# NoelShin/zutis

Hardware: AMD Instinct MI355X
Metric: images/sec, COCO2017-val-shaped ViT-B/16 dense semantic segmentation @336px (ZUTIS forward + semantic predict), batches of 32 per GPU, 3 independent batches in flight (higher is better)
Workload: dtype f16x3 (fp32-class)

## Files before the change

include/zutis_hip.h:

```cpp
#ifndef ZUTIS_HIP_H
#define ZUTIS_HIP_H

#include <stddef.h>

#ifdef __cplusplus
extern "C" {
#endif

typedef struct ihipStream_t* zh_stream_t;

#define ZH_OK 0
#define ZH_ERR_ARG (-1)
#define ZH_ERR_HIP (-2)
#define ZH_ERR_WORKSPACE (-3)

#define ZH_ACT_NONE 0
#define ZH_ACT_QUICKGELU 1
#define ZH_ACT_RELU 2
#define ZH_ACT_SIGMOID 3
#define ZH_ACT_GELU_ERF 4

#define ZH_ABI_VERSION 233
int zh_version(void);
const char* zh_arch(void);
const char* zh_last_error(void);

int zh_dev_set_gemm_overrides(int group_m, int tile, int tile_small);

int zh_dev_set_gemm_persist(int workgroups);

int zh_gemm_f16(const void* A, long lda, long strideA, const void* W, long ldw, long strideW,
                void* C, long ldc, long strideC, int out_f16,
                const float* bias, const float* residual, long ldr, long strideR, int res_rows,
                const void* pos_y, const void* pos_x, long ld_pos, int pos_h, int pos_w, int pos_f16,
                int act, int M, int N, int K, int batch, zh_stream_t stream);

int zh_gemm_f16_res16(const void* A, long lda, long strideA, const void* W, long ldw, long strideW,
                      void* C, long ldc, long strideC,
                      const float* bias, const void* residual, long ldr, long strideR, int res_rows,
                      int M, int N, int K, int batch, zh_stream_t stream);

#define ZH_GEMM_FIXED_K_ORDER 1
int zh_gemm_f16x3(const void* A, long lda, long strideA, long planeA, const void* W, long ldw, long strideW, long planeW,
                  void* C, long ldc, long strideC, long planeC, int out_kind, float out_scale,
                  const float* bias, const float* residual, long ldr, long strideR, int res_rows,
                  const void* pos_y, const void* pos_x, long ld_pos, int pos_h, int pos_w, int pos_f16,
                  int act, int M, int N, int K, int batch, int flags, zh_stream_t stream);

size_t zh_attention_splitk_workspace_size(int batch, int heads, int Tq, int head_dim, int ksplit);
int zh_attention_f16_splitk(const void* Q, long ldq, long strideQ, const void* K, long ldk, long strideK,
                            const void* V, long ldv, long strideV, void* O, long ldo, long strideO,
                            int batch, int heads, int Tq, int Tk, int head_dim, float scale,
                            long planeQ, long planeK, long planeV, long planeO, int ksplit, void* workspace, size_t workspace_bytes,
                            zh_stream_t stream);
int zh_attention_f16(const void* Q, long ldq, long strideQ, const void* K, long ldk, long strideK,
                     const void* V, long ldv, long strideV, void* O, long ldo, long strideO,
                     int batch, int heads, int Tq, int Tk, int head_dim, float scale,
                     long planeQ, long planeK, long planeV, long planeO, zh_stream_t stream);

int zh_attention_causal_f16(const void* Q, long ldq, long strideQ, const void* K, long ldk, long strideK,
                            const void* V, long ldv, long strideV, void* O, long ldo, long strideO,
                            int batch, int heads, int T, int head_dim, float scale,
                            long planeQ, long planeK, long planeV, long planeO, zh_stream_t stream);

int zh_embed_tokens_f32(const long long* tokens, const float* table, const float* pos, float* out, long n, int ctx, int D,
                        int vocab, zh_stream_t stream);
int zh_eot_rows_f32(const long long* tokens, const float* x, float* out, long n, int ctx, int D, zh_stream_t stream);
int zh_group_mean_l2norm(const float* x, float* out, int groups, int T, int E, zh_stream_t stream);

int zh_layernorm_f32(const float* x, long in_group_rows, long in_group_stride, long in_offset,
                     long out_group_rows, long out_group_stride, long out_offset,
                     const float* gamma, const float* beta, float eps,
                     float* out_f32, void* out_f16, void* out_f16_plus, float* out_f32_plus,
                     const float* add, int add_rows, int rows, int D, long lo_plane, int* status, zh_stream_t stream);
int zh_layernorm_f16(const void* x, long in_group_rows, long in_group_stride, long in_offset,
                     long out_group_rows, long out_group_stride, long out_offset,
                     const float* gamma, const float* beta, float eps,
                     float* out_f32, void* out_f16, void* out_f16_plus, float* out_f32_plus,
                     const float* add, int add_rows, int rows, int D, long lo_plane, int* status, zh_stream_t stream);
#define ZH_STATUS_RANGE 1
#define ZH_STATUS_NONFINITE 2
#define ZH_STATUS_LABEL 4

int zh_sum_layernorm_f32(const float* parts, int n_parts, long part_stride, const float* bias, const float* residual,
                         float* out_sum, const float* gamma, const float* beta, float eps,
                         float* out_f32, void* out_f16, long lo_plane,
                         long out_group_rows, long out_group_stride, long out_offset, int skip_first_in_group,
                         const float* gamma2, const float* beta2, float eps2, float* out2_f32, void* out2_f16, long lo_plane2,
                         long out2_group_rows, long out2_group_stride, long out2_offset,
                         int rows, int D, int* status, zh_stream_t stream);

int zh_assemble_tokens_ln(const float* patch_emb, const float* class_embedding, const float* pos_embed,
                          const float* gamma, const float* beta, float eps, float* out,
                          int B, int T, int D, zh_stream_t stream);

int zh_assemble_tokens_ln_f16(const float* patch_emb, const float* class_embedding, const float* pos_embed,
                              const float* gamma, const float* beta, float eps, void* out,
                              int B, int T, int D, zh_stream_t stream);

int zh_l2norm_rows(const float* x, float* out_f32, void* out_f16, float eps, int rows, int D, long lo_plane, float f16_scale, zh_stream_t stream);

size_t zh_global_ln_l2_workspace_size(int B, int M, int C);
int zh_global_ln_l2(const float* x, float* out_f32, void* out_f16, float eps, float l2_eps,
                    int B, int M, int C, void* workspace, size_t workspace_bytes, long lo_plane, float f16_scale, int* status,
                    zh_stream_t stream);

int zh_im2col_f16(const float* x, void* out, int B, int Cin, int H, int W, int patch, int Kpad, int pad_to_patch,
                  long lo_plane, zh_stream_t stream);

int zh_posembed_bicubic(const float* pos, float* out, int grid, int h, int w, int D, float scale_h, float scale_w,
                        int has_cls, zh_stream_t stream);

int zh_upsample2x_bilinear_cl(const float* x, float* out_f32, void* out_f16, int B, int h, int w, int D, long lo_plane,
                              int relu, zh_stream_t stream);

int zh_sine_pe(float* out, int h, int w, int D, float temperature, zh_stream_t stream);

int zh_add_rowperiodic_f16(const void* a, const float* add, void* out, long rows, int D, int add_rows, long a_lo_plane,
                           long lo_plane, zh_stream_t stream);

int zh_fill_f32(float* x, float value, long n, zh_stream_t stream);

int zh_cast_f32_f16(const float* x, const float* add, int add_rows, void* out, long rows, int D, long lo_plane, float f16_scale,
                    zh_stream_t stream);

int zh_upsample_argmax(const float* logits_lo, long long* labels, int B, int n, int h, int w, int H, int W,
                       float scale_h, float scale_w, zh_stream_t stream);

#define ZH_GT_U8 0
#define ZH_GT_RG16 1
int zh_upsample_argmax_score(const float* logits_lo, const unsigned char* gt, int gt_format, long long* hist_accum,
                             long long* labels, int B, int n, int h, int w, int H, int W, float scale_h, float scale_w,
                             zh_stream_t stream);

int zh_upsample_argmax_bytes(const float* logits_lo, unsigned char* labels_out, int label_format, unsigned char* overlay_out,
                             const unsigned char* packed, const int* desc, const unsigned char* palette, int alpha,
                             int B, int n, int h, int w, int H, int W, float scale_h, float scale_w, zh_stream_t stream);

int zh_upsample_bilinear_nchw(const float* x, float* out, unsigned char* mask_u8, float threshold, long planes,
                              int h, int w, int H, int W, float scale_h, float scale_w, zh_stream_t stream);

int zh_select_upsample_mask(const float* objectness, const float* masks, unsigned char* out_u8, long long* index, int B, int Q,
                            int h, int w, int H, int W, float scale_h, float scale_w, float threshold, zh_stream_t stream);

int zh_resize_nearest_u8(const unsigned char* x, unsigned char* out, int h, int w, int H, int W, float scale_h, float scale_w,
                         zh_stream_t stream);

int zh_confusion_hist(const long long* label_true, const long long* label_pred, long long* hist_accum, long total,
                      int n_class, zh_stream_t stream);

int zh_instance_mask_stats(const float* mask_proposals, long stride_image, float threshold, int B, int Q, int M,
                           float* sizes, float* confidence, unsigned char* binary, int* range_flag, zh_stream_t stream);
size_t zh_masked_mean_workspace_size(int B, int Q, int M, int E);
int zh_masked_mean_tokens(const float* tokens, const unsigned char* binary, const float* sizes, float* avg,
                          int B, int Q, int M, int E, void* workspace, size_t workspace_bytes, zh_stream_t stream);
int zh_instance_classify(const float* avg, const float* text, const float* confidence, float temperature,
                         int rows, int n_classes, int E, long long* category, float* score, zh_stream_t stream);
size_t zh_mask_iou_workspace_size(int n, long pixels);
int zh_mask_iou_counts(const unsigned char* masks, int n, long pixels, int* inter, int* uni,
                       void* workspace, size_t workspace_bytes, zh_stream_t stream);

#define ZH_RCN_KMAX 152
int zh_resize_crop_normalize_u8(const unsigned char* packed, long packed_bytes, const int* desc, int B, int n_px, int kmax,
                                const float* lut, float* out, zh_stream_t stream);
#define ZH_FILTER_BILINEAR 2
#define ZH_FILTER_BICUBIC 3
int zh_resize_normalize_u8(const unsigned char* packed, long packed_bytes, const int* desc, int B, int out_h, int out_w, int filter,
                           int kmax, const float* lut, float* out, zh_stream_t stream);

int zh_denormalize_u8(const float* x, unsigned char* rgb, int H, int W, const float* mean3, const float* std3,
                      zh_stream_t stream);
int zh_bgrid_coords(const unsigned char* rgb, int H, int W, double sigma_spatial, double sigma_luma, double sigma_chroma,
                    int* coords, zh_stream_t stream);
size_t zh_bilateral_workspace_size(int H, int W, double sigma_spatial, double sigma_luma, double sigma_chroma);
int zh_bilateral_solve(const unsigned char* rgb, const unsigned char* target_u8, const double* target_f64, int H, int W,
                       double sigma_spatial, double sigma_luma, double sigma_chroma, double confidence, double lam,
                       double a_diag_min, double cg_tol, int cg_maxiter, double* out_soft, int* stats,
                       double* n_out, double* m_out, void* workspace, size_t workspace_bytes, zh_stream_t stream);

int zh_bilateral_solve_batch(const unsigned char* rgb, const unsigned char* target_u8, const double* target_f64, int B, int H, int W,
                             double sigma_spatial, double sigma_luma, double sigma_chroma, double confidence, double lam,
                             double a_diag_min, double cg_tol, int cg_maxiter, double* out_soft, int* stats,
                             double* n_out, double* m_out, void* workspace, size_t workspace_bytes, zh_stream_t stream);

int zh_threshold_f64_u8(const double* x, double threshold, unsigned char* out, long n, zh_stream_t stream);

int zh_topk_rows(const float* scores, long ld, int rows, long N, int k, const long long* idx_map, long long idx_add,
                 long long* idx_out, float* val_out, long out_ld, zh_stream_t stream);

int zh_mask_nms(const int* inter, const int* uni, const float* scores, const long long* category_ids, int B, int Q,
                int nms_type, double nms_threshold, double sigma, double score_threshold,
                int* out_index, double* out_score, long long* out_category, int* out_count, double* packed, const int* range_flag,
                int* zero_word, zh_stream_t stream);

size_t zh_mask_runs_workspace_size(int n, int W);
int zh_mask_runs(const unsigned char* masks, const int* sel, int n_sel, int H, int W, int max_runs,
                 int* positions, int* nruns, int* box_area, void* workspace, size_t workspace_bytes, zh_stream_t stream);
int zh_mask_runs_kept(const unsigned char* masks, const int* kept_index, const int* kept_count, int B, int Q, int H, int W, int max_runs,
                      int* positions, long packed_capacity, int* nruns, int* box_area, void* workspace, size_t workspace_bytes,
                      zh_stream_t stream);

int zh_mask_rle_kept(const int* positions, long packed_capacity, const int* nruns, const int* kept_count, int B, int Q, int max_runs, long HW,
                     unsigned char* out, long out_capacity, int* out_len, zh_stream_t stream);

int zh_mask_rle_fused_supported(int H, int W, int max_runs);
int zh_mask_rle_fused_kept(const unsigned char* masks, const unsigned long long* bits, const int* kept_index, const int* kept_count, int B, int Q,
                           int H, int W, int max_runs, unsigned char* out, long out_capacity, int* cursor, int* info, zh_stream_t stream);

size_t zh_mask_match_cost_workspace_size(int B, int L, int Q, int H, int n_max);
int zh_mask_match_cost(const float* proposals, const unsigned char* gt_u8, const int* inst_off, float* costs, float* stat_p,
                       float* stat_pg, float* stat_g, int* skip, int* status, int B, int L, int Q, int h, int w, int H, int W,
                       int n_max, float weight_dice, float weight_bce, float scale_h, float scale_w, void* workspace,
                       size_t workspace_bytes, zh_stream_t stream);
int zh_mask_match_grad(const float* proposals, const unsigned char* gt_u8, const int* inst_off, const int* pairs, int n_pairs,
                       const float* stat_p, const float* stat_pg, const float* stat_g, const float* grad_out, float* grad_proposals,
                       int B, int L, int Q, int h, int w, int H, int W, float weight_dice, float weight_bce, float loss_scale,
                       float scale_h, float scale_w, zh_stream_t stream);
size_t zh_upsample_ce_workspace_size(int B, int H, int W);
int zh_upsample_ce_fwd(const float* logits_lo, const long long* labels, float* lse, float* out, int* status, int B, int n_cat,
                       int h, int w, int H, int W, int ignore_index, float scale_h, float scale_w, void* workspace,
                       size_t workspace_bytes, zh_stream_t stream);
int zh_upsample_ce_bwd(const float* logits_lo, const long long* labels, const float* lse, const float* ce_out,
                       const float* grad_out, float* grad_logits_lo, int B, int n_cat, int h, int w, int H, int W,
                       int ignore_index, float scale_h, float scale_w, zh_stream_t stream);
int zh_gemm_f32_strided(const float* A, long sAb, long sAm, long sAk, const float* Bm, long sBb, long sBn, long sBk, float* C,
                        long sCb, long sCm, long sCn, int batch, int M, int N, int K, zh_stream_t stream);

int zh_linear_assignment_max_dim(void);
size_t zh_linear_assignment_workspace_size(int B, int L, int n_tot);
int zh_linear_assignment(const float* costs, const int* inst_off, const int* skip, int B, int L, int Q, int n_max, int n_tot,
                         int* pairs, int* n_pairs, float* mask_loss, int* status, void* workspace, size_t workspace_bytes,
                         zh_stream_t stream);
int zh_pack_masks_u8(const void* const* src, const int* counts, int B, int elem_size, long HW, unsigned char* gt_u8, int* inst_off,
                     zh_stream_t stream);

int zh_plan_run(const void* cmds, int n, zh_stream_t stream);
int zh_plan_run2(const void* cmds_a, int na, zh_stream_t stream_a, const void* cmds_b, int nb, zh_stream_t stream_b);
int zh_plan_run_multi(const void* const* cmds, const int* n, const zh_stream_t* streams, int count);
const char* zh_plan_op_name(int op);

long zh_rle_counts_to_string_host(const long long* counts, long n, char* out, long cap);
long zh_rle_from_transitions_host(const int* positions, long stride, int packed, const int* nruns, long n, long HW, char* out, long cap,
                                  long long* offsets);

int zh_synth_geometry_u8(const unsigned char* packed, long packed_bytes, const int* desc, int N, int C, int ignore_index, int kmax,
                         int fill_w, int fill_h, int* work, unsigned char* out_rgbm, zh_stream_t stream);
int zh_synth_photometric_u8(unsigned char* rgbm, const int* desc, int N, int C, int* work, zh_stream_t stream);
int zh_synth_blur_u8(const unsigned char* rgbm, const int* desc, const float* weights, int N, int C, int ksize, unsigned char* out_rgbm,
                     zh_stream_t stream);
int zh_synth_compose(const unsigned char* rgbm, const unsigned char* rgbm_blurred, const int* desc, const int* samples, const int* work,
                     const float* lut, int N, int B, int C, int ignore_index, float* image, long long* semantic, unsigned char* onehot,
                     zh_stream_t stream);

long zh_rle_encode_host(const unsigned char* mask, int H, int W, char* out, long cap);

#ifdef __cplusplus
}
#endif
#endif
```

zutis_amd/build.py:

```python
from __future__ import annotations

import os
import subprocess
import sys

HERE = os.path.dirname(os.path.abspath(__file__))
CSRC = os.path.join(HERE, "csrc")
LIB = os.path.join(HERE, "libzutis_hip.so")
EXTRA_FLAGS = {"bilateral.hip": ["-ffp-contract=off"], "preprocess.hip": ["-ffp-contract=off"],
               "synth.hip": ["-ffp-contract=off"]}
NO_SCRATCH = {"gemm.hip", "gemm_x3.hip", "attention.hip", "preprocess.hip", "synth.hip", "resample.hip"}
MAX_SCRATCH = int(os.environ.get("ZH_BUILD_MAX_SCRATCH", "0"))
MIN_OCCUPANCY = {"attention.hip": {"attn_f16_kernelILi64ELi4ELi1ELi0EE": 3, "attn_f16_kernelILi64ELi4ELi0ELi0EE": 3,
                                   "attn_f16_kernelILi64ELi4ELi1ELi1EE": 2, "attn_f16_kernelILi96ELi4ELi1ELi0EE": 2,
                                   "attn_f16_kernelILi96ELi4ELi0ELi0EE": 2, "attn_f16_kernelILi96ELi4ELi1ELi1EE": 2},
                 "resample.hip": {"upsample_argmax_pk_kernelI7UaBytes": 3, "upsample_argmax_lds_kernelI7UaBytes": 6,
                                  "upsample_argmax_kernelI7UaBytes": 8}}
SOURCES = ["capi.hip", "gemm.hip", "gemm_x3.hip", "attention.hip", "norm.hip", "resample.hip", "metrics.hip", "instance.hip", "bilateral.hip", "preprocess.hip", "retrieval.hip", "text.hip", "criterion.hip", "assign.hip", "synth.hip", "plan.hip"]


def _hipcc() -> str:
    for c in (os.environ.get("HIPCC"), "/opt/rocm/bin/hipcc", "hipcc"):
        if c and (os.path.isabs(c) and os.path.exists(c) or not os.path.isabs(c)):
            return c
    raise RuntimeError("hipcc not found")


def sources():
    return [os.path.join(CSRC, s) for s in SOURCES if os.path.exists(os.path.join(CSRC, s))]


def needs_build() -> bool:
    if not os.path.exists(LIB):
        return True
    t = os.path.getmtime(LIB)
    deps = sources() + [os.path.join(CSRC, "common.h"), os.path.join(CSRC, "gemm_kernel.h"), os.path.join(CSRC, "gemm_skinny.h"),
                        os.path.join(CSRC, "rcn.h"), os.path.join(os.path.dirname(HERE), "include", "zutis_hip.h")]
    return any(os.path.getmtime(d) > t for d in deps)


def build(force: bool = False, verbose: bool = True) -> str:
    if not force and not needs_build():
        return LIB
    objs = []
    os.makedirs(os.path.join(HERE, "_obj"), exist_ok=True)
    from . import plan
    plan.generate_dispatch(os.path.join(CSRC, "plan_gen.inc"))
    procs = []
    for src in sources():
        obj = os.path.join(HERE, "_obj", os.path.basename(src)[:-4] + ".o")
        objs.append(obj)
        deps = [src, os.path.join(CSRC, "common.h")]
        if os.path.basename(src).startswith("gemm"):
            deps.append(os.path.join(CSRC, "gemm_kernel.h"))
            deps.append(os.path.join(CSRC, "gemm_skinny.h"))
        if os.path.basename(src) in ("preprocess.hip", "synth.hip"):
            deps.append(os.path.join(CSRC, "rcn.h"))
        if os.path.basename(src) in ("plan.hip", "capi.hip"):
            deps.append(os.path.join(os.path.dirname(HERE), "include", "zutis_hip.h"))
        if not force and os.path.exists(obj) and all(os.path.getmtime(obj) > os.path.getmtime(d) for d in deps):
            continue
        cmd = [_hipcc(), "--offload-arch=gfx950", "-O3", "-fPIC", "-std=c++17"] + EXTRA_FLAGS.get(os.path.basename(src), []) + \
              ["-c", src, "-o", obj]
        if os.path.basename(src) in NO_SCRATCH:
            cmd.insert(1, "-Rpass-analysis=kernel-resource-usage")
        if verbose:
            print(" ".join(cmd), flush=True)
        procs.append((cmd, src, subprocess.Popen(cmd, stderr=subprocess.PIPE, text=True)))
    for cmd, src, p in procs:
        _, err = p.communicate()
        if p.returncode != 0:
            sys.stderr.write(err)
            raise RuntimeError("hipcc failed: " + " ".join(cmd))
        if os.path.basename(src) in NO_SCRATCH:
            spills = [ln for ln in err.splitlines() if "ScratchSize [bytes/lane]:" in ln
                      and int(ln.split("ScratchSize [bytes/lane]:")[1].split()[0]) > MAX_SCRATCH]
            if spills:
                raise RuntimeError(f"{os.path.basename(src)}: a kernel spills to scratch (register budget exceeded): {spills[0].strip()}")
            fn = None
            min_occ = MIN_OCCUPANCY.get(os.path.basename(src), {})
            matched = set()
            for ln in err.splitlines():
                if "Function Name:" in ln:
                    fn = ln.split("Function Name:")[1].split()[0]
                elif "Occupancy [waves/SIMD]:" in ln and fn:
                    occ = int(ln.split("Occupancy [waves/SIMD]:")[1].split()[0])
                    for key, need in min_occ.items():
                        if key in fn:
                            matched.add(key)
                            if occ < need:
                                raise RuntimeError(f"{os.path.basename(src)}: {fn} compiles to {occ} waves/SIMD, its design needs {need}")
            unmatched = sorted(set(min_occ) - matched)
            if unmatched:
                raise RuntimeError(f"{os.path.basename(src)}: MIN_OCCUPANCY names no kernel of the compiler's remarks: {', '.join(unmatched)}")
        else:
            sys.stderr.write(err)
    cmd = [_hipcc(), "--offload-arch=gfx950", "-shared", "-fPIC", "-o", LIB] + objs
    if verbose:
        print(" ".join(cmd), flush=True)
    subprocess.check_call(cmd)
    return LIB


if __name__ == "__main__":
    print(build(force="--force" in sys.argv))
```

zutis_amd/csrc/attention.hip:

```cpp
#include "common.h"
#include <type_traits>

struct AttnArgs {
  const half_t* Q; long ldq, sQ;
  const half_t* K; long ldk, sK;
  const half_t* V; long ldv, sV;
  half_t* O; long ldo, sO;
  int Tq, Tk, H, nqb, groups;
  float scale_log2;
  int causal;
  long planeQ, planeK, planeV, planeO;
  int ksplit, kchunk;
  float* part_o; float* part_m; float* part_l;
};

typedef __fp16 fp16x4 __attribute__((__vector_size__(4 * sizeof(__fp16))));
typedef __attribute__((address_space(3))) fp16x4* lds_fp16x4_ptr;

#define KT 64
#define VS 96

#define ZH_ATTN_LAZY_LOG2 8.0f

__device__ __forceinline__ float zh_xor32_max(float x) {
  float a = x, b = x;
  asm volatile("s_nop 1\n\tv_permlane32_swap_b32 %0, %1" : "+v"(a), "+v"(b));
  float r;
  asm("v_max_f32 %0, %1, %2" : "=v"(r) : "v"(a), "v"(b));
  return r;
}
__device__ __forceinline__ float zh_xor32_sum(float x) {
  float a = x, b = x;
  asm volatile("s_nop 1\n\tv_permlane32_swap_b32 %0, %1" : "+v"(a), "+v"(b));
  return a + b;
}

template <int DH, int NWAVE, int X3, int PIPE>
__global__ __launch_bounds__(64 * NWAVE, X3 ? 2 : (DH == 64 ? 3 : 2)) void attn_f16_kernel(AttnArgs p) {
  static_assert(!PIPE || X3, "the pipelined loop exists for the split-pair kernels");
  constexpr int NT = 64 * NWAVE;
  constexpr int KS = DH + 8;
  constexpr int NKS = DH / 16;
  constexpr int NDT = DH / 32;
  constexpr int CPR = DH / 8;
  constexpr int KTT = X3 ? 32 : KT;
  constexpr int NU = KTT / 32;
  constexpr int NLD = (KTT * CPR + NT - 1) / NT;
  constexpr bool LDFULL = (KTT * CPR) % NT == 0;
  __shared__ __attribute__((aligned(16))) half_t sKb[2][KTT * KS];
  __shared__ __attribute__((aligned(16))) half_t sKl[X3 ? 2 : 1][X3 ? KTT * KS : 8];
  __shared__ __attribute__((aligned(16))) half_t sVb[2][KTT * VS];
  __shared__ __attribute__((aligned(16))) half_t sVl[X3 ? 2 : 1][X3 ? KTT * VS : 8];

  const int tid = threadIdx.x, lane = tid & 63, wave = tid >> 6;
  const int id = blockIdx.y * gridDim.x + blockIdx.x;
  const int per_group = p.nqb * p.ksplit;
  const int item = (id & 7) * (int)(gridDim.x >> 3) + (id >> 3);
  if (item >= p.groups * per_group) return;
  const int group = item / per_group;
  const int qbs = item - group * per_group;
  const int qb = qbs / p.ksplit, ks = qbs - qb * p.ksplit;
  const int head = group % p.H, img = group / p.H;
  const int q0 = qb * (32 * NWAVE) + wave * 32;
  const int ql = lane & 31, hh = lane >> 5;
  const long hoff = (long)head * DH;

  const int key0 = ks * p.kchunk;
  const int key_end = p.ksplit > 1 ? min(p.Tk, key0 + p.kchunk) : p.Tk;
  const half_t* Q = p.Q + (long)img * p.sQ + hoff;
  const half_t* K = p.K + (long)img * p.sK + hoff;
  const half_t* V = p.V + (long)img * p.sV + hoff;

  half8_t qf[NKS], qfl[X3 ? NKS : 1];
  const half_t* qp = Q + (long)min(q0 + ql, p.Tq - 1) * p.ldq + 8 * hh;
#pragma unroll
  for (int ks = 0; ks < NKS; ++ks) qf[ks] = *(const half8_t*)(qp + 16 * ks);
  if (X3) {
#pragma unroll
    for (int ks = 0; ks < NKS; ++ks) qfl[ks] = *(const half8_t*)(qp + p.planeQ + 16 * ks);
  }

  f32x16 oacc[NDT];
#pragma unroll
  for (int d = 0; d < NDT; ++d)
#pragma unroll
    for (int r = 0; r < 16; ++r) oacc[d][r] = 0.f;
  float m_run = -INFINITY;
  f32x16 lacc;
#pragma unroll
  for (int r = 0; r < 16; ++r) lacc[r] = 0.f;
  float l_run = 0.f;
  half8_t ones;
#pragma unroll
  for (int i = 0; i < 8; ++i) ones[i] = (half_t)1.0f;

  struct TileRegs { half8_t k[NLD], v[NLD], kl[X3 ? NLD : 1], vl[X3 ? NLD : 1]; };
  TileRegs ra;
  const unsigned ldk2 = (unsigned)p.ldk * 2u, ldv2 = (unsigned)p.ldv * 2u;
  const char* const Kl = (const char*)(K + p.planeK);
  const char* const Vl = (const char*)(V + p.planeV);
  auto load_k = [&](int kbase, TileRegs& r) {
#pragma unroll
    for (int i = 0; i < NLD; ++i) {
      const int c = tid + i * NT;
      const int row = c / CPR, cc = c - row * CPR;
      if (LDFULL || c < KTT * CPR) {
        const unsigned ok = (unsigned)min(kbase + row, key_end - 1) * ldk2 + (unsigned)cc * 16u;
        r.k[i] = *(const half8_t*)((const char*)K + ok);
        if (X3) r.kl[i] = *(const half8_t*)(Kl + ok);
      }
    }
  };
  auto load_v = [&](int kbase, TileRegs& r) {
#pragma unroll
    for (int i = 0; i < NLD; ++i) {
      const int c = tid + i * NT;
      const int row = c / CPR, cc = c - row * CPR;
      if (LDFULL || c < KTT * CPR) {
        const unsigned ov = (unsigned)min(kbase + row, key_end - 1) * ldv2 + (unsigned)cc * 16u;
        r.v[i] = *(const half8_t*)((const char*)V + ov);
        if (X3) r.vl[i] = *(const half8_t*)(Vl + ov);
      }
    }
  };
  auto store_k = [&](int buf, const TileRegs& r) {
#pragma unroll
    for (int i = 0; i < NLD; ++i) {
      const int c = tid + i * NT;
      const int row = c / CPR, cc = c - row * CPR;
      if (LDFULL || c < KTT * CPR) {
        *(half8_t*)(sKb[buf] + row * KS + cc * 8) = r.k[i];
        if (X3) *(half8_t*)(sKl[buf] + row * KS + cc * 8) = r.kl[i];
      }
    }
  };
  auto store_v = [&](int buf, const TileRegs& r) {
#pragma unroll
    for (int i = 0; i < NLD; ++i) {
      const int c = tid + i * NT;
      const int row = c / CPR, cc = c - row * CPR;
      if (LDFULL || c < KTT * CPR) {
        *(half8_t*)(sVb[buf] + row * VS + cc * 8) = r.v[i];
        if (X3) *(half8_t*)(sVl[buf] + row * VS + cc * 8) = r.vl[i];
      }
    }
  };

  const int krow = (ql & 0x13) | ((ql & 4) << 1) | ((ql & 8) >> 1);
  const int tr_row = 8 * hh + ((lane & 15) >> 2);
  const int tr_col = 16 * ((lane >> 4) & 1) + 4 * (lane & 3);

  int ntiles = (max(key_end - key0, 0) + KTT - 1) / KTT;
  if (p.causal) {
    const int qlast = min(p.Tq, (qb + 1) * (32 * NWAVE)) - 1;
    ntiles = min(ntiles, qlast / KTT + 1);
  }
  const int qidx = q0 + ql;
  const bool active = q0 < p.Tq;

  auto qk = [&](int t, f32x16 (&s)[NU]) {
    const half_t* sK = sKb[t & 1];
#pragma unroll
    for (int u = 0; u < NU; ++u) {
#pragma unroll
      for (int r = 0; r < 16; ++r) s[u][r] = 0.f;
      const half_t* kp = sK + (32 * u + krow) * KS + 8 * hh;
#pragma unroll
      for (int ks = 0; ks < NKS; ++ks) {
        half8_t kf = *(const half8_t*)(kp + 16 * ks);
        half8_t kl;
        if (X3) kl = *(const half8_t*)(sKl[t & 1] + (32 * u + krow) * KS + 8 * hh + 16 * ks);
        s[u] = __builtin_amdgcn_mfma_f32_32x32x16_f16(kf, qf[ks], s[u], 0, 0, 0);
        if (X3) {
          s[u] = __builtin_amdgcn_mfma_f32_32x32x16_f16(kl, qf[ks], s[u], 0, 0, 0);
          s[u] = __builtin_amdgcn_mfma_f32_32x32x16_f16(kf, qfl[ks], s[u], 0, 0, 0);
        }
      }
    }
  };
  typedef unsigned u32x4 __attribute__((ext_vector_type(4)));
  struct PFrag { u32x4 hi[NU][2], lo[X3 ? NU : 1][2]; };
  auto softmax = [&](int t, f32x16 (&s)[NU], PFrag& P, auto masked) {
    constexpr bool MASKED = decltype(masked)::value;
    const int kbase = key0 + t * KTT;
    float mx = -INFINITY;
    if (MASKED && (kbase + KTT > key_end || (p.causal && kbase + KTT - 1 > q0))) {
#pragma unroll
      for (int u = 0; u < NU; ++u)
#pragma unroll
        for (int r = 0; r < 16; ++r) {
          const int key = kbase + 32 * u + 16 * (r >> 3) + 8 * hh + (r & 7);
          if (key >= key_end || (p.causal && key > qidx)) s[u][r] = -INFINITY;
        }
    }
    {
      float m4[4] = {mx, mx, mx, mx};
#pragma unroll
      for (int u = 0; u < NU; ++u)
#pragma unroll
        for (int r = 0; r < 16; r += 8) {
          m4[0] = fmaxf(fmaxf(m4[0], s[u][r + 0]), s[u][r + 1]);
          m4[1] = fmaxf(fmaxf(m4[1], s[u][r + 2]), s[u][r + 3]);
          m4[2] = fmaxf(fmaxf(m4[2], s[u][r + 4]), s[u][r + 5]);
          m4[3] = fmaxf(fmaxf(m4[3], s[u][r + 6]), s[u][r + 7]);
        }
      mx = fmaxf(fmaxf(m4[0], m4[1]), fmaxf(m4[2], m4[3]));
    }
    mx = zh_xor32_max(mx);
    const float m_cand = mx * p.scale_log2;
    const float m_new = m_cand > m_run + ZH_ATTN_LAZY_LOG2 ? m_cand : m_run;
    const float alpha = __builtin_amdgcn_exp2f(m_run - m_new);
    m_run = m_new;
    float lsum2[2] = {0.f, 0.f};
#pragma unroll
    for (int u = 0; u < NU; ++u)
#pragma unroll
      for (int r = 0; r < 16; r += 2) {
        const float e0 = __builtin_amdgcn_exp2f(__builtin_fmaf(s[u][r], p.scale_log2, -m_new));
        const float e1 = __builtin_amdgcn_exp2f(__builtin_fmaf(s[u][r + 1], p.scale_log2, -m_new));
        if (X3) { lsum2[0] += e0; lsum2[1] += e1; }
        const half2_t eh2 = {(half_t)e0, (half_t)e1};
        unsigned eh = __builtin_bit_cast(unsigned, eh2);
        if (X3) {
          unsigned el;
          asm("v_fma_mixlo_f16 %0, -%1, 1.0, %2 op_sel:[0,0,0] op_sel_hi:[1,0,0]\n\t"
              "v_fma_mixhi_f16 %0, -%1, 1.0, %3 op_sel:[1,0,0] op_sel_hi:[1,0,0]"
              : "=&v"(el) : "v"(eh), "v"(e0), "v"(e1));
          P.lo[u][r >> 3][(r >> 1) & 3] = el;
        }
        P.hi[u][r >> 3][(r >> 1) & 3] = eh;
      }
    if (__any(alpha != 1.0f)) {
#pragma unroll
      for (int d = 0; d < NDT; ++d)
#pragma unroll
        for (int r = 0; r < 16; ++r) oacc[d][r] *= alpha;
      if (!X3) {
#pragma unroll
        for (int r = 0; r < 16; ++r) lacc[r] *= alpha;
      }
    }
    if (X3) l_run = l_run * alpha + (lsum2[0] + lsum2[1]);
  };
  auto pv = [&](int t, const PFrag& P) {
    const half_t* sV = sVb[t & 1];
#pragma unroll
    for (int u = 0; u < NU; ++u)
#pragma unroll
      for (int ks = 0; ks < 2; ++ks) {
        if (!X3) lacc = __builtin_amdgcn_mfma_f32_32x32x16_f16(ones, __builtin_bit_cast(half8_t, P.hi[u][ks]), lacc, 0, 0, 0);
        const half_t* vp = sV + (32 * u + 16 * ks + tr_row) * VS + tr_col;
#pragma unroll
        for (int d = 0; d < NDT; ++d) {
          fp16x4 lo = __builtin_amdgcn_ds_read_tr16_b64_v4f16((lds_fp16x4_ptr)(vp + 32 * d));
          fp16x4 hi = __builtin_amdgcn_ds_read_tr16_b64_v4f16((lds_fp16x4_ptr)(vp + 32 * d + 4 * VS));
          half8_t vf;
          __builtin_memcpy(&vf, &lo, 8);
          __builtin_memcpy(((char*)&vf) + 8, &hi, 8);
          half8_t vl;
          if (X3) {
            const half_t* vq = sVl[t & 1] + (32 * u + 16 * ks + tr_row) * VS + tr_col;
            fp16x4 llo = __builtin_amdgcn_ds_read_tr16_b64_v4f16((lds_fp16x4_ptr)(vq + 32 * d));
            fp16x4 lhi = __builtin_amdgcn_ds_read_tr16_b64_v4f16((lds_fp16x4_ptr)(vq + 32 * d + 4 * VS));
            __builtin_memcpy(&vl, &llo, 8);
            __builtin_memcpy(((char*)&vl) + 8, &lhi, 8);
          }
          const half8_t pf = __builtin_bit_cast(half8_t, P.hi[u][ks]);
          oacc[d] = __builtin_amdgcn_mfma_f32_32x32x16_f16(vf, pf, oacc[d], 0, 0, 0);
          if (X3) {
            oacc[d] = __builtin_amdgcn_mfma_f32_32x32x16_f16(vl, pf, oacc[d], 0, 0, 0);
            oacc[d] = __builtin_amdgcn_mfma_f32_32x32x16_f16(vf, __builtin_bit_cast(half8_t, P.lo[u][ks]), oacc[d], 0, 0, 0);
          }
        }
      }
  };

  if (PIPE && !p.causal) {
    load_k(key0, ra);
    load_v(key0, ra);
    store_k(0, ra);
    store_v(0, ra);
    if (ntiles > 1) { load_k(key0 + KTT, ra); store_k(1, ra); }
    __syncthreads();
    f32x16 sA[NU], sB[NU];
    PFrag P;
    if (active) qk(0, sA);
    __syncthreads();
    auto step = [&](int t, auto par, f32x16 (&cur)[NU], f32x16 (&nxt)[NU]) {
      constexpr int PAR = decltype(par)::value;
      if (t + 2 < ntiles) load_k(key0 + (t + 2) * KTT, ra);
      load_v(key0 + (t + 1) * KTT, ra);
      if (active) {
        qk(PAR ^ 1, nxt);
        softmax(t, cur, P, std::false_type{});
        pv(PAR, P);
      }
      if (t + 2 < ntiles) store_k(PAR, ra);
      store_v(PAR ^ 1, ra);
      __syncthreads();
    };
    int t = 0;
    for (; t + 2 < ntiles; t += 2) {
      step(t, std::integral_constant<int, 0>{}, sA, sB);
      step(t + 1, std::integral_constant<int, 1>{}, sB, sA);
    }
    if (t + 1 < ntiles) {
      step(t, std::integral_constant<int, 0>{}, sA, sB);
      if (active) { softmax(t + 1, sB, P, std::true_type{}); pv(1, P); }
    } else if (active) {
      softmax(t, sA, P, std::true_type{});
      pv(0, P);
    }
  } else {
  auto load_tile = [&](int kbase, TileRegs& r) { load_k(kbase, r); load_v(kbase, r); };
  auto store_tile = [&](int buf, const TileRegs& r) { store_k(buf, r); store_v(buf, r); };
  load_tile(key0, ra);
  store_tile(0, ra);
  __syncthreads();
  auto compute = [&](int t) {
    if (active) {
      f32x16 s[NU];
      PFrag P;
      qk(t, s);
      softmax(t, s, P, std::true_type{});
      pv(t, P);
    }
  };

  for (int t = 0; t < ntiles; t += 2) {
    if (t + 1 < ntiles) load_tile(key0 + (t + 1) * KTT, ra);
    compute(t);
    if (t + 1 < ntiles) store_tile(1, ra);
    __syncthreads();
    if (t + 1 >= ntiles) break;
    if (t + 2 < ntiles) load_tile(key0 + (t + 2) * KTT, ra);
    compute(t + 1);
    if (t + 2 < ntiles) store_tile(0, ra);
    __syncthreads();
  }
  }

  for (int once = 0; once < 1; ++once) {
  const float l_row = X3 ? zh_xor32_sum(l_run) : lacc[0];
  const int qr = q0 + ql;
  if (p.ksplit > 1) {
    if (qr < p.Tq) {
      float* po = p.part_o + (((long)ks * (p.groups / p.H) + img) * p.Tq + qr) * ((long)p.H * DH) + hoff + 4 * hh;
#pragma unroll
      for (int d = 0; d < NDT; ++d)
#pragma unroll
        for (int g = 0; g < 4; ++g)
          *(f32x4*)(po + 32 * d + 8 * g) = (f32x4){oacc[d][4 * g], oacc[d][4 * g + 1], oacc[d][4 * g + 2], oacc[d][4 * g + 3]};
      if (hh == 0) {
        const long mi = ((long)ks * p.groups + group) * p.Tq + qr;
        p.part_m[mi] = m_run;
        p.part_l[mi] = l_row;
      }
    }
    continue;
  }
  const float inv = 1.0f / l_row;
  if (qr < p.Tq) {
    half_t* op = p.O + (long)img * p.sO + (long)qr * p.ldo + hoff + 4 * hh;
#pragma unroll
    for (int d = 0; d < NDT; ++d)
#pragma unroll
      for (int g = 0; g < 4; ++g) {
        const f32x4 o = {oacc[d][4 * g] * inv, oacc[d][4 * g + 1] * inv, oacc[d][4 * g + 2] * inv, oacc[d][4 * g + 3] * inv};
        zh_store_h4(op + 32 * d + 8 * g, p.planeO, o);
      }
  }
  }
}

__global__ __launch_bounds__(256) void attn_combine_kernel(const float* part_o, const float* part_m, const float* part_l, half_t* O, long ldo, long sO,
                                                           long planeO, int S, int B, int H, int Tq, int DH) {
  const int D = H * DH, c4 = D / 4;
  const long i = (long)blockIdx.x * 256 + threadIdx.x;
  if (i >= (long)B * Tq * c4) return;
  const int col = (int)(i % c4) * 4;
  const long row = i / c4;
  const int img = (int)(row / Tq), q = (int)(row - (long)img * Tq), head = col / DH;
  float m = -INFINITY;
  for (int s = 0; s < S; ++s) m = fmaxf(m, part_m[(((long)s * B + img) * H + head) * Tq + q]);
  f32x4 acc = {0.f, 0.f, 0.f, 0.f};
  float l = 0.f;
  for (int s = 0; s < S; ++s) {
    const long mi = (((long)s * B + img) * H + head) * Tq + q;
    const float w = __builtin_amdgcn_exp2f(part_m[mi] - m);
    l += w * part_l[mi];
    acc += *(const f32x4*)(part_o + (((long)s * B + img) * Tq + q) * D + col) * w;
  }
  const float inv = 1.0f / l;
  zh_store_h4(O + (long)img * sO + (long)q * ldo + col, planeO, acc * inv);
}

static int attention_launch(const void* Q, long ldq, long strideQ, const void* K, long ldk, long strideK,
                            const void* V, long ldv, long strideV, void* O, long ldo, long strideO,
                            int batch, int heads, int Tq, int Tk, int head_dim, float scale, int causal,
                            long planeQ, long planeK, long planeV, long planeO, hipStream_t stream, int ksplit = 1, void* workspace = nullptr,
                            size_t workspace_bytes = 0) {
  ZH_CHECK_ARG(Q && K && V && O, "zh_attention_f16: null operand");
  ZH_CHECK_ARG(batch > 0 && heads > 0 && Tq > 0 && Tk > 0, "zh_attention_f16: bad shape");
  ZH_CHECK_ARG(head_dim == 64 || head_dim == 96, "zh_attention_f16: head_dim %d not in {64, 96}", head_dim);
  ZH_CHECK_ARG(ldq % 8 == 0 && ldk % 8 == 0 && ldv % 8 == 0 && ldo % 4 == 0 && strideQ % 8 == 0 && strideK % 8 == 0 &&
                   strideV % 8 == 0 && strideO % 4 == 0 && planeQ % 8 == 0 && planeK % 8 == 0 && planeV % 8 == 0 && planeO % 4 == 0,
               "zh_attention_f16: row/batch/plane strides must keep 16-byte (Q,K,V) / 8-byte (O) alignment");
  ZH_CHECK_ARG(((uintptr_t)Q & 15) == 0 && ((uintptr_t)K & 15) == 0 && ((uintptr_t)V & 15) == 0 && ((uintptr_t)O & 7) == 0,
               "zh_attention_f16: misaligned pointer");
  ZH_CHECK_ARG(heads < 65536 && batch < 65536, "zh_attention_f16: heads/batch exceed grid limits");
  ZH_CHECK_ARG((long)Tk * ldk * 2 < (1L << 32) && (long)Tk * ldv * 2 < (1L << 32), "zh_attention_f16: Tk * ldk (ldv) exceeds 2^31 elements");
  ZH_CHECK_ARG((planeQ != 0) == (planeK != 0) && (planeQ != 0) == (planeV != 0),
               "zh_attention_f16: the split-pair mode needs the lo planes of Q, K and V (all three or none)");
  AttnArgs p;
  p.Q = (const half_t*)Q; p.ldq = ldq; p.sQ = strideQ;
  p.K = (const half_t*)K; p.ldk = ldk; p.sK = strideK;
  p.V = (const half_t*)V; p.ldv = ldv; p.sV = strideV;
  p.O = (half_t*)O; p.ldo = ldo; p.sO = strideO;
  p.Tq = Tq; p.Tk = Tk; p.H = heads;
  p.scale_log2 = scale * 1.4426950408889634f;
  p.causal = causal;
  p.planeQ = planeQ; p.planeK = planeK; p.planeV = planeV; p.planeO = planeO;
  const bool x3 = planeQ != 0;
  p.nqb = zh_cdiv(Tq, 128);
  p.groups = heads * batch;
  p.ksplit = 1; p.kchunk = 0; p.part_o = p.part_m = p.part_l = nullptr;
  if (ksplit > 1) {
    ZH_CHECK_ARG(!causal && ksplit <= 64, "zh_attention_f16_splitk: ksplit %d not in 1..64 (and not for the causal form)", ksplit);
    const int ktt = x3 ? 32 : 64;
    p.ksplit = ksplit;
    p.kchunk = zh_cdiv(zh_cdiv(Tk, ktt), ksplit) * ktt;
    ZH_CHECK_ARG((long)(ksplit - 1) * p.kchunk < Tk, "zh_attention_f16_splitk: ksplit %d leaves an empty key chunk for Tk = %d", ksplit, Tk);
    const size_t no = (size_t)ksplit * batch * Tq * heads * head_dim, nm = (size_t)ksplit * batch * heads * Tq;
    ZH_CHECK_ARG(workspace && workspace_bytes >= (no + 2 * nm) * 4 && ((uintptr_t)workspace & 15) == 0,
                 "zh_attention_f16_splitk: workspace too small or misaligned (%zu < %zu)", workspace_bytes, (no + 2 * nm) * 4);
    p.part_o = (float*)workspace; p.part_m = p.part_o + no; p.part_l = p.part_m + nm;
  }
  const long items = (long)p.groups * p.nqb * p.ksplit;
  ZH_CHECK_ARG(items < (1L << 31) - 8, "zh_attention_f16: grid too large");
  const long nblk = (long)zh_cdiv(items, 8) * 8;
  ZH_CHECK_ARG(nblk < (1L << 31), "zh_attention_f16: grid too large");
  dim3 grid((unsigned)nblk);
  const bool pipe = x3 && (head_dim == 96 || zh_cdiv(nblk, 512L) <= zh_cdiv(nblk, 768L));
  if (head_dim == 64) {
    if (x3 && pipe) hipLaunchKernelGGL((attn_f16_kernel<64, 4, 1, 1>), grid, dim3(256), 0, stream, p);
    else if (x3) hipLaunchKernelGGL((attn_f16_kernel<64, 4, 1, 0>), grid, dim3(256), 0, stream, p);
    else hipLaunchKernelGGL((attn_f16_kernel<64, 4, 0, 0>), grid, dim3(256), 0, stream, p);
  } else {
    if (x3 && pipe) hipLaunchKernelGGL((attn_f16_kernel<96, 4, 1, 1>), grid, dim3(256), 0, stream, p);
    else if (x3) hipLaunchKernelGGL((attn_f16_kernel<96, 4, 1, 0>), grid, dim3(256), 0, stream, p);
    else hipLaunchKernelGGL((attn_f16_kernel<96, 4, 0, 0>), grid, dim3(256), 0, stream, p);
  }
  ZH_CHECK_LAUNCH("zh_attention_f16");
  if (p.ksplit > 1) {
    const long n4 = (long)batch * Tq * heads * head_dim / 4;
    hipLaunchKernelGGL(attn_combine_kernel, dim3((unsigned)zh_cdiv(n4, 256)), dim3(256), 0, stream, p.part_o, p.part_m, p.part_l, p.O, ldo, strideO,
                       planeO, p.ksplit, batch, heads, Tq, head_dim);
    ZH_CHECK_LAUNCH("zh_attention_f16_splitk (combine)");
  }
  return ZH_OK;
}

extern "C" size_t zh_attention_splitk_workspace_size(int batch, int heads, int Tq, int head_dim, int ksplit) {
  return ((size_t)ksplit * batch * Tq * heads * head_dim + 2 * (size_t)ksplit * batch * heads * Tq) * 4;
}
extern "C" int zh_attention_f16_splitk(const void* Q, long ldq, long strideQ, const void* K, long ldk, long strideK,
                                       const void* V, long ldv, long strideV, void* O, long ldo, long strideO,
                                       int batch, int heads, int Tq, int Tk, int head_dim, float scale,
                                       long planeQ, long planeK, long planeV, long planeO, int ksplit, void* workspace, size_t workspace_bytes,
                                       hipStream_t stream) {
  return attention_launch(Q, ldq, strideQ, K, ldk, strideK, V, ldv, strideV, O, ldo, strideO, batch, heads, Tq, Tk, head_dim,
                          scale, 0, planeQ, planeK, planeV, planeO, stream, ksplit, workspace, workspace_bytes);
}

extern "C" int zh_attention_f16(const void* Q, long ldq, long strideQ, const void* K, long ldk, long strideK,
                                const void* V, long ldv, long strideV, void* O, long ldo, long strideO,
                                int batch, int heads, int Tq, int Tk, int head_dim, float scale,
                                long planeQ, long planeK, long planeV, long planeO, hipStream_t stream) {
  return attention_launch(Q, ldq, strideQ, K, ldk, strideK, V, ldv, strideV, O, ldo, strideO, batch, heads, Tq, Tk, head_dim,
                          scale, 0, planeQ, planeK, planeV, planeO, stream);
}

extern "C" int zh_attention_causal_f16(const void* Q, long ldq, long strideQ, const void* K, long ldk, long strideK,
                                       const void* V, long ldv, long strideV, void* O, long ldo, long strideO,
                                       int batch, int heads, int T, int head_dim, float scale,
                                       long planeQ, long planeK, long planeV, long planeO, hipStream_t stream) {
  return attention_launch(Q, ldq, strideQ, K, ldk, strideK, V, ldv, strideV, O, ldo, strideO, batch, heads, T, T, head_dim,
                          scale, 1, planeQ, planeK, planeV, planeO, stream);
}
```

Before: 2949.

## Stage split-pair attention K/V tiles via global_load_lds DMA with XOR-swizzled LDS

Adds a DMA template variant of the split-pair (f16x3) attention kernel. It loads K and V hi/lo planes straight from global memory into LDS with global_load_lds_dwordx4, so the data no longer passes through registers and a separate LDS store. The padded row stride is replaced by an XOR chunk swizzle to avoid bank conflicts, and waitcnt calls before each barrier wait for the DMA. This is meant to free VGPRs and issue slots in the attention inner loop. The cost is more address arithmetic per LDS read, added inline-asm complexity, and a register-staging fallback kept behind a new debug knob.

```diff
diff --git a/include/zutis_hip.h b/include/zutis_hip.h
--- a/include/zutis_hip.h
+++ b/include/zutis_hip.h
@@ -20,7 +20,7 @@
 #define ZH_ACT_SIGMOID 3
 #define ZH_ACT_GELU_ERF 4
 
-#define ZH_ABI_VERSION 233
+#define ZH_ABI_VERSION 234
 int zh_version(void);
 const char* zh_arch(void);
 const char* zh_last_error(void);
@@ -28,6 +28,9 @@
 int zh_dev_set_gemm_overrides(int group_m, int tile, int tile_small);
 
 int zh_dev_set_gemm_persist(int workgroups);
+
+int zh_dev_set_attention_staging(int force_registers);
+int zh_attention_lds_offset(int head_dim, int row, int chunk);
 
 int zh_gemm_f16(const void* A, long lda, long strideA, const void* W, long ldw, long strideW,
                 void* C, long ldc, long strideC, int out_f16,
diff --git a/zutis_amd/build.py b/zutis_amd/build.py
--- a/zutis_amd/build.py
+++ b/zutis_amd/build.py
@@ -11,9 +11,11 @@
                "synth.hip": ["-ffp-contract=off"]}
 NO_SCRATCH = {"gemm.hip", "gemm_x3.hip", "attention.hip", "preprocess.hip", "synth.hip", "resample.hip"}
 MAX_SCRATCH = int(os.environ.get("ZH_BUILD_MAX_SCRATCH", "0"))
-MIN_OCCUPANCY = {"attention.hip": {"attn_f16_kernelILi64ELi4ELi1ELi0EE": 3, "attn_f16_kernelILi64ELi4ELi0ELi0EE": 3,
-                                   "attn_f16_kernelILi64ELi4ELi1ELi1EE": 2, "attn_f16_kernelILi96ELi4ELi1ELi0EE": 2,
-                                   "attn_f16_kernelILi96ELi4ELi0ELi0EE": 2, "attn_f16_kernelILi96ELi4ELi1ELi1EE": 2},
+MIN_OCCUPANCY = {"attention.hip": {"attn_f16_kernelILi64ELi4ELi1ELi0ELi0EE": 3, "attn_f16_kernelILi64ELi4ELi0ELi0ELi0EE": 3,
+                                   "attn_f16_kernelILi64ELi4ELi1ELi1ELi0EE": 2, "attn_f16_kernelILi96ELi4ELi1ELi0ELi0EE": 2,
+                                   "attn_f16_kernelILi96ELi4ELi0ELi0ELi0EE": 2, "attn_f16_kernelILi96ELi4ELi1ELi1ELi0EE": 2,
+                                   "attn_f16_kernelILi64ELi4ELi1ELi0ELi1EE": 3, "attn_f16_kernelILi64ELi4ELi1ELi1ELi1EE": 2,
+                                   "attn_f16_kernelILi96ELi4ELi1ELi0ELi1EE": 2, "attn_f16_kernelILi96ELi4ELi1ELi1ELi1EE": 2},
                  "resample.hip": {"upsample_argmax_pk_kernelI7UaBytes": 3, "upsample_argmax_lds_kernelI7UaBytes": 6,
                                   "upsample_argmax_kernelI7UaBytes": 8}}
 SOURCES = ["capi.hip", "gemm.hip", "gemm_x3.hip", "attention.hip", "norm.hip", "resample.hip", "metrics.hip", "instance.hip", "bilateral.hip", "preprocess.hip", "retrieval.hip", "text.hip", "criterion.hip", "assign.hip", "synth.hip", "plan.hip"]
diff --git a/zutis_amd/csrc/attention.hip b/zutis_amd/csrc/attention.hip
--- a/zutis_amd/csrc/attention.hip
+++ b/zutis_amd/csrc/attention.hip
@@ -35,11 +35,17 @@
   return a + b;
 }
 
-template <int DH, int NWAVE, int X3, int PIPE>
+__host__ __device__ constexpr int zh_attn_lds_chunk(int dh, int row, int chunk) {
+  return dh == 64 ? chunk ^ ((((row >> 1) & 1) << 2) | ((row >> 2) & 3)) : chunk ^ ((row >> 2) & 3);
+}
+
+template <int DH, int NWAVE, int X3, int PIPE, int DMA>
 __global__ __launch_bounds__(64 * NWAVE, X3 ? 2 : (DH == 64 ? 3 : 2)) void attn_f16_kernel(AttnArgs p) {
   static_assert(!PIPE || X3, "the pipelined loop exists for the split-pair kernels");
+  static_assert(!DMA || X3, "LDS-DMA staging exists for the split-pair kernels");
   constexpr int NT = 64 * NWAVE;
-  constexpr int KS = DH + 8;
+  constexpr int KS = DMA ? DH : DH + 8;
+  constexpr int VST = DMA ? DH : VS;
   constexpr int NKS = DH / 16;
   constexpr int NDT = DH / 32;
   constexpr int CPR = DH / 8;
@@ -49,8 +55,8 @@
   constexpr bool LDFULL = (KTT * CPR) % NT == 0;
   __shared__ __attribute__((aligned(16))) half_t sKb[2][KTT * KS];
   __shared__ __attribute__((aligned(16))) half_t sKl[X3 ? 2 : 1][X3 ? KTT * KS : 8];
-  __shared__ __attribute__((aligned(16))) half_t sVb[2][KTT * VS];
-  __shared__ __attribute__((aligned(16))) half_t sVl[X3 ? 2 : 1][X3 ? KTT * VS : 8];
+  __shared__ __attribute__((aligned(16))) half_t sVb[2][KTT * VST];
+  __shared__ __attribute__((aligned(16))) half_t sVl[X3 ? 2 : 1][X3 ? KTT * VST : 8];
 
   const int tid = threadIdx.x, lane = tid & 63, wave = tid >> 6;
   const int id = blockIdx.y * gridDim.x + blockIdx.x;
@@ -99,7 +105,35 @@
   const unsigned ldk2 = (unsigned)p.ldk * 2u, ldv2 = (unsigned)p.ldv * 2u;
   const char* const Kl = (const char*)(K + p.planeK);
   const char* const Vl = (const char*)(V + p.planeV);
-  auto load_k = [&](int kbase, TileRegs& r) {
+  constexpr int PIECES = KTT * CPR / 64, NP = (PIECES + NWAVE - 1) / NWAVE;
+  static_assert(!DMA || (KTT * CPR) % 64 == 0, "whole 1-KiB pieces");
+  int dma_row[NP]; unsigned dma_col[NP], dma_lds[NP];
+#pragma unroll
+  for (int i = 0; i < NP; ++i) {
+    const int pc = min(wave + i * NWAVE, PIECES - 1);
+    const int slot = pc * 64 + lane;
+    dma_row[i] = slot / CPR;
+    dma_col[i] = (unsigned)zh_attn_lds_chunk(DH, dma_row[i], slot - dma_row[i] * CPR) * 16u;
+    dma_lds[i] = (unsigned)__builtin_amdgcn_readfirstlane(pc * 1024);
+  }
+  auto dma_plane = [&](const char* gbase, const half_t* lds, unsigned ld2, int kbase) {
+    const uintptr_t gb = (uintptr_t)gbase;
+    const char* sb = (const char*)(((uintptr_t)(unsigned)__builtin_amdgcn_readfirstlane((int)(gb >> 32)) << 32) |
+                                   (uintptr_t)(unsigned)__builtin_amdgcn_readfirstlane((int)(unsigned)gb));
+#pragma unroll
+    for (int i = 0; i < NP; ++i) {
+      const unsigned off = (unsigned)min(kbase + dma_row[i], key_end - 1) * ld2 + dma_col[i];
+      asm volatile("s_mov_b32 m0, %0\n\ts_nop 0\n\tglobal_load_lds_dwordx4 %1, %2"
+                   :: "s"((unsigned)(uintptr_t)lds + dma_lds[i]), "v"(off), "s"(sb) : "memory");
+    }
+  };
+  auto dma_wait = [&]() { if (DMA) { __builtin_amdgcn_s_waitcnt(0x0F70); asm volatile("" ::: "memory"); } };
+  auto load_k = [&](int kbase, int buf, TileRegs& r) {
+    if constexpr (DMA) {
+      dma_plane((const char*)K, sKb[buf], ldk2, kbase);
+      dma_plane(Kl, sKl[buf], ldk2, kbase);
+      return;
+    }
 #pragma unroll
     for (int i = 0; i < NLD; ++i) {
       const int c = tid + i * NT;
@@ -111,7 +145,12 @@
       }
     }
   };
-  auto load_v = [&](int kbase, TileRegs& r) {
+  auto load_v = [&](int kbase, int buf, TileRegs& r) {
+    if constexpr (DMA) {
+      dma_plane((const char*)V, sVb[buf], ldv2, kbase);
+      dma_plane(Vl, sVl[buf], ldv2, kbase);
+      return;
+    }
 #pragma unroll
     for (int i = 0; i < NLD; ++i) {
       const int c = tid + i * NT;
@@ -124,6 +163,7 @@
     }
   };
   auto store_k = [&](int buf, const TileRegs& r) {
+    if constexpr (DMA) return;
 #pragma unroll
     for (int i = 0; i < NLD; ++i) {
       const int c = tid + i * NT;
@@ -135,13 +175,14 @@
     }
   };
   auto store_v = [&](int buf, const TileRegs& r) {
+    if constexpr (DMA) return;
 #pragma unroll
     for (int i = 0; i < NLD; ++i) {
       const int c = tid + i * NT;
       const int row = c / CPR, cc = c - row * CPR;
       if (LDFULL || c < KTT * CPR) {
-        *(half8_t*)(sVb[buf] + row * VS + cc * 8) = r.v[i];
-        if (X3) *(half8_t*)(sVl[buf] + row * VS + cc * 8) = r.vl[i];
+        *(half8_t*)(sVb[buf] + row * VST + cc * 8) = r.v[i];
+        if (X3) *(half8_t*)(sVl[buf] + row * VST + cc * 8) = r.vl[i];
       }
     }
   };
@@ -149,6 +190,8 @@
   const int krow = (ql & 0x13) | ((ql & 4) << 1) | ((ql & 8) >> 1);
   const int tr_row = 8 * hh + ((lane & 15) >> 2);
   const int tr_col = 16 * ((lane >> 4) & 1) + 4 * (lane & 3);
+
+  auto lds_off = [&](int row, int col) { return row * DH + zh_attn_lds_chunk(DH, row, col >> 3) * 8 + (col & 7); };
 
   int ntiles = (max(key_end - key0, 0) + KTT - 1) / KTT;
   if (p.causal) {
@@ -167,9 +210,15 @@
       const half_t* kp = sK + (32 * u + krow) * KS + 8 * hh;
 #pragma unroll
       for (int ks = 0; ks < NKS; ++ks) {
-        half8_t kf = *(const half8_t*)(kp + 16 * ks);
-        half8_t kl;
-        if (X3) kl = *(const half8_t*)(sKl[t & 1] + (32 * u + krow) * KS + 8 * hh + 16 * ks);
+        half8_t kf, kl;
+        if constexpr (DMA) {
+          const int ko = lds_off(32 * u + krow, 8 * hh + 16 * ks);
+          kf = *(const half8_t*)(sK + ko);
+          kl = *(const half8_t*)(sKl[t & 1] + ko);
+        } else {
+          kf = *(const half8_t*)(kp + 16 * ks);
+          if (X3) kl = *(const half8_t*)(sKl[t & 1] + (32 * u + krow) * KS + 8 * hh + 16 * ks);
+        }
         s[u] = __builtin_amdgcn_mfma_f32_32x32x16_f16(kf, qf[ks], s[u], 0, 0, 0);
         if (X3) {
           s[u] = __builtin_amdgcn_mfma_f32_32x32x16_f16(kl, qf[ks], s[u], 0, 0, 0);
@@ -249,19 +298,21 @@
 #pragma unroll
       for (int ks = 0; ks < 2; ++ks) {
         if (!X3) lacc = __builtin_amdgcn_mfma_f32_32x32x16_f16(ones, __builtin_bit_cast(half8_t, P.hi[u][ks]), lacc, 0, 0, 0);
-        const half_t* vp = sV + (32 * u + 16 * ks + tr_row) * VS + tr_col;
+        const int vr = 32 * u + 16 * ks + tr_row;
+        const half_t* vp = sV + vr * VST + tr_col;
 #pragma unroll
         for (int d = 0; d < NDT; ++d) {
-          fp16x4 lo = __builtin_amdgcn_ds_read_tr16_b64_v4f16((lds_fp16x4_ptr)(vp + 32 * d));
-          fp16x4 hi = __builtin_amdgcn_ds_read_tr16_b64_v4f16((lds_fp16x4_ptr)(vp + 32 * d + 4 * VS));
+          const int vo0 = DMA ? lds_off(vr, tr_col + 32 * d) : 0, vo1 = DMA ? lds_off(vr + 4, tr_col + 32 * d) : 0;
+          fp16x4 lo = __builtin_amdgcn_ds_read_tr16_b64_v4f16((lds_fp16x4_ptr)(DMA ? sV + vo0 : vp + 32 * d));
+          fp16x4 hi = __builtin_amdgcn_ds_read_tr16_b64_v4f16((lds_fp16x4_ptr)(DMA ? sV + vo1 : vp + 32 * d + 4 * VST));
           half8_t vf;
           __builtin_memcpy(&vf, &lo, 8);
           __builtin_memcpy(((char*)&vf) + 8, &hi, 8);
           half8_t vl;
           if (X3) {
-            const half_t* vq = sVl[t & 1] + (32 * u + 16 * ks + tr_row) * VS + tr_col;
-            fp16x4 llo = __builtin_amdgcn_ds_read_tr16_b64_v4f16((lds_fp16x4_ptr)(vq + 32 * d));
-            fp16x4 lhi = __builtin_amdgcn_ds_read_tr16_b64_v4f16((lds_fp16x4_ptr)(vq + 32 * d + 4 * VS));
+            const half_t* vq = sVl[t & 1] + (DMA ? 0 : vr * VST + tr_col);
+            fp16x4 llo = __builtin_amdgcn_ds_read_tr16_b64_v4f16((lds_fp16x4_ptr)(DMA ? vq + vo0 : vq + 32 * d));
+            fp16x4 lhi = __builtin_amdgcn_ds_read_tr16_b64_v4f16((lds_fp16x4_ptr)(DMA ? vq + vo1 : vq + 32 * d + 4 * VST));
             __builtin_memcpy(&vl, &llo, 8);
             __builtin_memcpy(((char*)&vl) + 8, &lhi, 8);
           }
@@ -276,11 +327,12 @@
   };
 
   if (PIPE && !p.causal) {
-    load_k(key0, ra);
-    load_v(key0, ra);
+    load_k(key0, 0, ra);
+    load_v(key0, 0, ra);
     store_k(0, ra);
     store_v(0, ra);
-    if (ntiles > 1) { load_k(key0 + KTT, ra); store_k(1, ra); }
+    if (ntiles > 1) { load_k(key0 + KTT, 1, ra); store_k(1, ra); }
+    dma_wait();
     __syncthreads();
     f32x16 sA[NU], sB[NU];
     PFrag P;
@@ -288,8 +340,8 @@
     __syncthreads();
     auto step = [&](int t, auto par, f32x16 (&cur)[NU], f32x16 (&nxt)[NU]) {
       constexpr int PAR = decltype(par)::value;
-      if (t + 2 < ntiles) load_k(key0 + (t + 2) * KTT, ra);
-      load_v(key0 + (t + 1) * KTT, ra);
+      if (t + 2 < ntiles) load_k(key0 + (t + 2) * KTT, PAR, ra);
+      load_v(key0 + (t + 1) * KTT, PAR ^ 1, ra);
       if (active) {
         qk(PAR ^ 1, nxt);
         softmax(t, cur, P, std::false_type{});
@@ -297,6 +349,7 @@
       }
       if (t + 2 < ntiles) store_k(PAR, ra);
       store_v(PAR ^ 1, ra);
+      dma_wait();
       __syncthreads();
     };
     int t = 0;
@@ -312,10 +365,11 @@
       pv(0, P);
     }
   } else {
-  auto load_tile = [&](int kbase, TileRegs& r) { load_k(kbase, r); load_v(kbase, r); };
+  auto load_tile = [&](int kbase, int buf, TileRegs& r) { load_k(kbase, buf, r); load_v(kbase, buf, r); };
   auto store_tile = [&](int buf, const TileRegs& r) { store_k(buf, r); store_v(buf, r); };
-  load_tile(key0, ra);
+  load_tile(key0, 0, ra);
   store_tile(0, ra);
+  dma_wait();
   __syncthreads();
   auto compute = [&](int t) {
     if (active) {
@@ -328,14 +382,16 @@
   };
 
   for (int t = 0; t < ntiles; t += 2) {
-    if (t + 1 < ntiles) load_tile(key0 + (t + 1) * KTT, ra);
+    if (t + 1 < ntiles) load_tile(key0 + (t + 1) * KTT, 1, ra);
     compute(t);
     if (t + 1 < ntiles) store_tile(1, ra);
+    dma_wait();
     __syncthreads();
     if (t + 1 >= ntiles) break;
-    if (t + 2 < ntiles) load_tile(key0 + (t + 2) * KTT, ra);
+    if (t + 2 < ntiles) load_tile(key0 + (t + 2) * KTT, 0, ra);
     compute(t + 1);
     if (t + 2 < ntiles) store_tile(0, ra);
+    dma_wait();
     __syncthreads();
   }
   }
@@ -395,6 +451,17 @@
   zh_store_h4(O + (long)img * sO + (long)q * ldo + col, planeO, acc * inv);
 }
 
+static int g_attn_force_regs = 0;
+extern "C" int zh_dev_set_attention_staging(int force_registers) {
+  ZH_CHECK_ARG(force_registers == 0 || force_registers == 1, "zh_dev_set_attention_staging: %d is not 0 (LDS-DMA where the operands allow it) or 1 (registers)", force_registers);
+  g_attn_force_regs = force_registers;
+  return ZH_OK;
+}
+extern "C" int zh_attention_lds_offset(int head_dim, int row, int chunk) {
+  if ((head_dim != 64 && head_dim != 96) || row < 0 || row >= 32 || chunk < 0 || chunk >= head_dim / 8) return -1;
+  return (row * (head_dim / 8) + zh_attn_lds_chunk(head_dim, row, chunk)) * 16;
+}
+
 static int attention_launch(const void* Q, long ldq, long strideQ, const void* K, long ldk, long strideK,
                             const void* V, long ldv, long strideV, void* O, long ldo, long strideO,
                             int batch, int heads, int Tq, int Tk, int head_dim, float scale, int causal,
@@ -406,7 +473,8 @@
   ZH_CHECK_ARG(ldq % 8 == 0 && ldk % 8 == 0 && ldv % 8 == 0 && ldo % 4 == 0 && strideQ % 8 == 0 && strideK % 8 == 0 &&
                    strideV % 8 == 0 && strideO % 4 == 0 && planeQ % 8 == 0 && planeK % 8 == 0 && planeV % 8 == 0 && planeO % 4 == 0,
                "zh_attention_f16: row/batch/plane strides must keep 16-byte (Q,K,V) / 8-byte (O) alignment");
-  ZH_CHECK_ARG(((uintptr_t)Q & 15) == 0 && ((uintptr_t)K & 15) == 0 && ((uintptr_t)V & 15) == 0 && ((uintptr_t)O & 7) == 0,
+  const uintptr_t kv_mask = planeQ != 0 ? 1 : 15;
+  ZH_CHECK_ARG(((uintptr_t)Q & 15) == 0 && ((uintptr_t)K & kv_mask) == 0 && ((uintptr_t)V & kv_mask) == 0 && ((uintptr_t)O & 7) == 0,
                "zh_attention_f16: misaligned pointer");
   ZH_CHECK_ARG(heads < 65536 && batch < 65536, "zh_attention_f16: heads/batch exceed grid limits");
   ZH_CHECK_ARG((long)Tk * ldk * 2 < (1L << 32) && (long)Tk * ldv * 2 < (1L << 32), "zh_attention_f16: Tk * ldk (ldv) exceeds 2^31 elements");
@@ -442,14 +510,19 @@
   ZH_CHECK_ARG(nblk < (1L << 31), "zh_attention_f16: grid too large");
   dim3 grid((unsigned)nblk);
   const bool pipe = x3 && (head_dim == 96 || zh_cdiv(nblk, 512L) <= zh_cdiv(nblk, 768L));
+  const bool dma = x3 && !g_attn_force_regs && (((uintptr_t)K | (uintptr_t)V) & 15) == 0;
   if (head_dim == 64) {
-    if (x3 && pipe) hipLaunchKernelGGL((attn_f16_kernel<64, 4, 1, 1>), grid, dim3(256), 0, stream, p);
-    else if (x3) hipLaunchKernelGGL((attn_f16_kernel<64, 4, 1, 0>), grid, dim3(256), 0, stream, p);
-    else hipLaunchKernelGGL((attn_f16_kernel<64, 4, 0, 0>), grid, dim3(256), 0, stream, p);
+    if (x3 && pipe && dma) hipLaunchKernelGGL((attn_f16_kernel<64, 4, 1, 1, 1>), grid, dim3(256), 0, stream, p);
+    else if (x3 && dma) hipLaunchKernelGGL((attn_f16_kernel<64, 4, 1, 0, 1>), grid, dim3(256), 0, stream, p);
+    else if (x3 && pipe) hipLaunchKernelGGL((attn_f16_kernel<64, 4, 1, 1, 0>), grid, dim3(256), 0, stream, p);
+    else if (x3) hipLaunchKernelGGL((attn_f16_kernel<64, 4, 1, 0, 0>), grid, dim3(256), 0, stream, p);
+    else hipLaunchKernelGGL((attn_f16_kernel<64, 4, 0, 0, 0>), grid, dim3(256), 0, stream, p);
   } else {
-    if (x3 && pipe) hipLaunchKernelGGL((attn_f16_kernel<96, 4, 1, 1>), grid, dim3(256), 0, stream, p);
-    else if (x3) hipLaunchKernelGGL((attn_f16_kernel<96, 4, 1, 0>), grid, dim3(256), 0, stream, p);
-    else hipLaunchKernelGGL((attn_f16_kernel<96, 4, 0, 0>), grid, dim3(256), 0, stream, p);
+    if (x3 && pipe && dma) hipLaunchKernelGGL((attn_f16_kernel<96, 4, 1, 1, 1>), grid, dim3(256), 0, stream, p);
+    else if (x3 && dma) hipLaunchKernelGGL((attn_f16_kernel<96, 4, 1, 0, 1>), grid, dim3(256), 0, stream, p);
+    else if (x3 && pipe) hipLaunchKernelGGL((attn_f16_kernel<96, 4, 1, 1, 0>), grid, dim3(256), 0, stream, p);
+    else if (x3) hipLaunchKernelGGL((attn_f16_kernel<96, 4, 1, 0, 0>), grid, dim3(256), 0, stream, p);
+    else hipLaunchKernelGGL((attn_f16_kernel<96, 4, 0, 0, 0>), grid, dim3(256), 0, stream, p);
   }
   ZH_CHECK_LAUNCH("zh_attention_f16");
   if (p.ksplit > 1) {
```

Result: no change. 2973, median of 6 (+0.8%).
